# criteo/tf-yarn

Measured on AMD Instinct MI355X. Metric: examples/sec (whole node), Criteo wide-and-deep, higher is better.
Workload: dtype bf16; 1 GPU; model=wide_and_deep_criteo, global_batch=65536, per_gpu_batch=65536, dense_features=13, sparse_features=26, embedding_dim=16, table_rows_per_feature=1000000, parallelism=dp1, alltoall_mode=unprobed

## Files before the change

setup.py:

```python

import os

os.environ.setdefault("PYTORCH_ROCM_ARCH", "gfx950")

from pybind11.setup_helpers import Pybind11Extension
from setuptools import find_packages, setup
from torch.utils.cpp_extension import (BuildExtension,
                                       CUDAExtension)

CSRC = os.path.join("tf_yarn_amd", "ops", "csrc")

kv_ext = Pybind11Extension(
    "tf_yarn_amd._kv_native",
    sources=[os.path.join("tf_yarn_amd", "csrc_kv", "kv_server.cpp")],
    cxx_std=17,
    extra_compile_args=["-O2", "-pthread"],
)

ext = CUDAExtension(
    name="tf_yarn_amd.ops._C",
    sources=[
        os.path.join(CSRC, "bindings.cpp"),
        os.path.join(CSRC, "fused_optimizers.hip"),
        os.path.join(CSRC, "embedding.hip"),
        os.path.join(CSRC, "binned_scatter.hip"),
        os.path.join(CSRC, "sparse_adagrad.hip"),
        os.path.join(CSRC, "elementwise.hip"),
        os.path.join(CSRC, "wgrad.hip"),
        os.path.join(CSRC, "gemm_bt.hip"),
        os.path.join(CSRC, "lt_linear.hip"),
        os.path.join(CSRC, "eval_metrics.hip"),
    ],
    extra_compile_args={
        "cxx": ["-O3"],
        "nvcc": ["-O3", "--offload-arch=gfx950"],
    },
    libraries=["hipblaslt"],
)

setup(
    name="tf_yarn_amd",
    version="0.1.0",
    description=("MI355X-native distributed-training launcher with "
                 "criteo/tf-yarn's capabilities"),
    packages=find_packages(include=["tf_yarn_amd", "tf_yarn_amd.*"]),
    package_data={"tf_yarn_amd": ["default.log.conf"]},
    python_requires=">=3.9",
    ext_modules=[ext, kv_ext],
    cmdclass={"build_ext": BuildExtension},
)
```

tf_yarn_amd/models/wide_deep.py:

```python

from __future__ import annotations

import logging
import math
from typing import List, NamedTuple, Optional, Tuple

import torch
import torch.distributed as dist
from torch import nn

from tf_yarn_amd import ops

logger = logging.getLogger(__name__)

CRITEO_DENSE = 13
CRITEO_SPARSE = 26
DEFAULT_TABLE_SIZES = [1_000_000] * CRITEO_SPARSE


SPARSE_OPTIMIZERS = ("sgd", "adagrad", "ftrl")
DEEP_SPARSE_OPTIMIZERS = SPARSE_OPTIMIZERS + ("rowwise_adagrad",)


def _check_sparse_rule(name: str, value: str, dim: int = 1) -> str:
# ... 343 lines not shown
                                all_ids.reshape(all_grads.numel(), -1),
                                all_grads, alpha=-lr / world)
        self._gathered = []

    @torch.no_grad()
    def apply_sparse_updates(self, lr: float, process_group=None) -> None:
        if not self._sink:
            return
        self.start_sparse_sync(process_group)
        self.finish_sparse_sync(lr)

    def clear_pending(self) -> None:
        self._sink.clear()
        self._gathered = []


class _DeepInput(torch.autograd.Function):

    DENSE_PAD = 16

    @staticmethod
    def forward(ctx, dense, table, flat_ids, dim, out_bf16, sink):
        b = dense.shape[0]
        f = flat_ids.numel() // b
        dtype = torch.bfloat16 if out_bf16 else torch.float32
        out = torch.empty(b, _DeepInput.DENSE_PAD + f * dim,
                          dtype=dtype, device=dense.device)
        out[:, :dense.shape[1]] = dense.to(dtype)
        out[:, dense.shape[1]:_DeepInput.DENSE_PAD] = 0
        ops.emb_fwd_into(table, flat_ids, out, _DeepInput.DENSE_PAD)
        ctx.sink = sink
        ctx.save_for_backward(flat_ids)
        return out

    @staticmethod
    def backward(ctx, grad_out):
        (flat_ids,) = ctx.saved_tensors
        emb_grad = grad_out[:, _DeepInput.DENSE_PAD:].contiguous()
        ctx.sink.append((flat_ids, emb_grad))
        return None, None, None, None, None, None


class ScalarHead(nn.Module):

    def __init__(self, in_features: int, dtype=torch.float32):
        super().__init__()
        bound = 1.0 / math.sqrt(in_features)
        self.weight = nn.Parameter(
            (torch.rand(in_features, dtype=torch.float32) * 2 - 1) * bound)
        self.bias = nn.Parameter(torch.zeros(1, dtype=torch.float32))
        if dtype != torch.float32:
            self.weight.data = self.weight.data.to(dtype)
            self.bias.data = self.bias.data.to(dtype)

    def forward(self, x):
        if x.size(-1) % 4 == 0:
            return ops.ScalarHeadFn.apply(x, self.weight, self.bias)
        if x.is_cuda:
            pad = (-x.size(-1)) % 4
            xp = nn.functional.pad(x, (0, pad))
            wp = nn.functional.pad(self.weight, (0, pad))
            return ops.ScalarHeadFn.apply(xp, wp, self.bias)
        return x @ self.weight + self.bias


class FusedLinearReLU(nn.Module):

    def __init__(self, in_features: int, out_features: int,
                 dtype=torch.float32):
        super().__init__()
        self.weight = nn.Parameter(
            torch.empty(out_features, in_features, dtype=dtype))
        self.bias = nn.Parameter(torch.zeros(out_features, dtype=dtype))
        nn.init.kaiming_uniform_(self.weight, a=math.sqrt(5))

    def forward(self, x):
        return ops.linear_bias_relu(x, self.weight, self.bias)


class WideAndDeep(nn.Module):

    def __init__(self,
                 dense_dim: int = CRITEO_DENSE,
                 table_sizes: Optional[List[int]] = None,
                 embedding_dim: int = 16,
                 hidden: Tuple[int, ...] = (1024, 512, 256),
                 compute_dtype: torch.dtype = torch.float32,
                 sharded: bool = False,
                 process_group=None,
                 sparse_optimizer: str = "sgd",
                 sparse_eps: float = 1e-10,
                 sparse_initial_accumulator: float = 0.0,
                 wide_sparse_optimizer: Optional[str] = None,
                 sparse_l1: float = 0.0, sparse_l2: float = 0.0,
                 wide_sparse_lr: Optional[float] = None):
        super().__init__()
        table_sizes = table_sizes or DEFAULT_TABLE_SIZES
        if wide_sparse_optimizer is None:
            wide_sparse_optimizer = _default_wide_rule(sparse_optimizer)
        sparse_kw = dict(
            sparse_optimizer=sparse_optimizer, sparse_eps=sparse_eps,
            sparse_initial_accumulator=sparse_initial_accumulator,
            sparse_l1=sparse_l1, sparse_l2=sparse_l2)
        self.sparse_optimizer = sparse_optimizer
        self.wide_sparse_optimizer = wide_sparse_optimizer
        self.compute_dtype = compute_dtype
        self.dense_dim = dense_dim
        bf16 = compute_dtype == torch.bfloat16
        self.sharded = sharded
        if sharded:
            from tf_yarn_amd.models.sharded_embedding import \
                ShardedCriteoEmbeddings
            self.embeddings = ShardedCriteoEmbeddings(
                table_sizes, embedding_dim, out_bf16=bf16,
                process_group=process_group,
                wide_sparse_optimizer=wide_sparse_optimizer,
                wide_sparse_lr=wide_sparse_lr, **sparse_kw)
            self.deep_embedding = None
            self.wide_embedding = None
        else:
            self.embeddings = None
            self.deep_embedding = SparseEmbedding(
                table_sizes, embedding_dim, out_bf16=bf16, **sparse_kw)
            wide_kw = dict(sparse_kw, sparse_optimizer=wide_sparse_optimizer,
                           wide_sparse_lr=wide_sparse_lr)
            self.wide_embedding = WideScalarEmbedding(table_sizes,
                                                      out_bf16=bf16,
                                                      **wide_kw)
        self.wide_dense = ScalarHead(dense_dim, compute_dtype)
        layers: List[nn.Module] = []
        in_dim = _DeepInput.DENSE_PAD + len(table_sizes) * embedding_dim
        for h in hidden:
            layers.append(FusedLinearReLU(in_dim, h))
            in_dim = h
        self.mlp = nn.Sequential(*layers)
        self.head = ScalarHead(in_dim, compute_dtype)
        if bf16:
            self.mlp = self.mlp.to(torch.bfloat16)

    def _deep_tower(self, deep_in: torch.Tensor) -> torch.Tensor:
        n = len(self.mlp)
        last = self.mlp[n - 1] if n else None
        head = self.head
        if not (isinstance(last, FusedLinearReLU) and deep_in.is_cuda
                and ops.HAVE_EXT and deep_in.dim() == 2
                and deep_in.dtype == torch.bfloat16
                and last.weight.dtype == torch.bfloat16
                and last.bias.dtype == torch.bfloat16
                and head.weight.dtype == torch.bfloat16
                and head.bias.dtype == torch.bfloat16
                and last.weight.shape[0] % 4 == 0
                and ops.fused_head_bwd_enabled()):
            return head(self.mlp(deep_in))
        h = deep_in
        for i in range(n - 1):
            h = self.mlp[i](h)
        return ops.linear_bias_relu_head(h, last.weight, last.bias,
                                         head.weight, head.bias)

    def forward(self, dense: torch.Tensor, sparse_ids: torch.Tensor,
                labels: Optional[torch.Tensor] = None) -> torch.Tensor:
        dense = dense.to(self.compute_dtype)
        if self.sharded:
            b = dense.shape[0]
            emb = self.embeddings
            deep_in = torch.empty(
                b, _DeepInput.DENSE_PAD + emb.F * emb.dim,
                dtype=self.compute_dtype, device=dense.device)
            deep_in, wide_sum = emb(sparse_ids, deep_in,
                                    _DeepInput.DENSE_PAD, dense=dense)
            deep_out = self._deep_tower(deep_in)
            wide_sum = wide_sum.to(deep_out.dtype)
            wd = self.wide_dense(dense)
            if labels is not None:
                return ops.bce_head_loss(deep_out, wide_sum, wd, labels)
            return deep_out + wide_sum + wd
        emb = self.deep_embedding
        flat = (sparse_ids + emb.offsets.unsqueeze(0)).reshape(-1)
        deep_in = _DeepInput.apply(
            dense, emb.weight, flat, emb.dim,
            self.compute_dtype == torch.bfloat16, emb._sink)
        deep_out = self._deep_tower(deep_in)
        wide_emb = self.wide_embedding(sparse_ids).to(deep_out.dtype)
        wd = self.wide_dense(dense)
        if labels is not None:
            return ops.bce_head_loss(deep_out, wide_emb, wd, labels)
        return deep_out + wide_emb + wd

    def start_sparse_sync(self, process_group=None) -> None:
        if self.sharded:
            return
        self.deep_embedding.start_sparse_sync(process_group)
        self.wide_embedding.start_sparse_sync(process_group)

    def finish_sparse_sync(self, lr: float, stream=None) -> None:
        if self.sharded:
            self.embeddings.apply_sparse_updates(lr, stream=stream)
            return
        self.deep_embedding.finish_sparse_sync(lr)
        self.wide_embedding.finish_sparse_sync(lr)

    def apply_sparse_updates(self, lr: float, process_group=None) -> None:
        self.start_sparse_sync(process_group)
        self.finish_sparse_sync(lr)

    def clear_pending(self) -> None:
        if self.sharded:
            self.embeddings.clear_pending()
            return
        self.deep_embedding.clear_pending()
        self.wide_embedding.clear_pending()


class FlatInputWideAndDeep(nn.Module):

    def __init__(self, dense_dim: int = CRITEO_DENSE,
                 table_sizes: Optional[List[int]] = None,
                 embedding_dim: int = 16,
                 hidden: Tuple[int, ...] = (1024, 512, 256),
                 compute_dtype: torch.dtype = torch.float32,
                 sharded: bool = False, process_group=None,
                 sparse_optimizer: str = "sgd", sparse_eps: float = 1e-10,
                 sparse_initial_accumulator: float = 0.0,
                 wide_sparse_optimizer: Optional[str] = None,
                 sparse_l1: float = 0.0, sparse_l2: float = 0.0,
                 wide_sparse_lr: Optional[float] = None):
        super().__init__()
        self.dense_dim = dense_dim
        init_acc = sparse_initial_accumulator
        self.net = WideAndDeep(dense_dim=dense_dim,
                               sparse_optimizer=sparse_optimizer,
                               sparse_eps=sparse_eps,
                               sparse_initial_accumulator=init_acc,
                               wide_sparse_optimizer=wide_sparse_optimizer,
                               sparse_l1=sparse_l1, sparse_l2=sparse_l2,
                               wide_sparse_lr=wide_sparse_lr,
                               table_sizes=table_sizes,
                               embedding_dim=embedding_dim, hidden=hidden,
                               compute_dtype=compute_dtype,
                               sharded=sharded,
                               process_group=process_group)

    def forward(self, x: torch.Tensor,
                labels: Optional[torch.Tensor] = None) -> torch.Tensor:
        dense = x[:, :self.dense_dim]
        ids = x[:, self.dense_dim:].long()
        return self.net(dense, ids, labels=labels)

    def start_sparse_sync(self, process_group=None) -> None:
        self.net.start_sparse_sync(process_group)

    def finish_sparse_sync(self, lr: float, stream=None) -> None:
        self.net.finish_sparse_sync(lr, stream=stream)

    def apply_sparse_updates(self, lr: float, process_group=None) -> None:
        self.net.apply_sparse_updates(lr, process_group)

    def clear_pending(self) -> None:
        self.net.clear_pending()
```

tf_yarn_amd/ops/__init__.py:

```python

from __future__ import annotations

import functools
import logging
import os
from typing import NamedTuple, Optional, Tuple

import torch

logger = logging.getLogger(__name__)

try:
    from tf_yarn_amd.ops import _C
    HAVE_EXT = True
except ImportError as _e:
    _C = None
    HAVE_EXT = False
    _IMPORT_ERROR = _e


def _require_ext() -> None:
    if not HAVE_EXT:
        raise RuntimeError(
            "tf_yarn_amd.ops._C is not built but a GPU tensor was passed. "
# ... 696 lines not shown
    return _env_switch_on("MIYARN_FUSED_HEAD_GRADS")


def col_reduce_dot_sum(x: torch.Tensor, dy: torch.Tensor,
                       out_dtype: torch.dtype = torch.float32):
    if _on_gpu(x, dy):
        _require_ext()
        if out_dtype in (torch.float32, torch.bfloat16):
            dw, db = _C.col_reduce_dot_sum(x.contiguous(), dy.contiguous(),
                                           out_dtype == torch.bfloat16)
            return dw, db
        dw, db = _C.col_reduce_dot_sum(x.contiguous(), dy.contiguous(),
                                       False)
        return dw.to(out_dtype), db.to(out_dtype)
    dw = (x.float() * dy.float().unsqueeze(1)).sum(dim=0)
    db = dy.float().sum().reshape(1)
    return dw.to(out_dtype), db.to(out_dtype)


def row_dot(x: torch.Tensor, w: torch.Tensor,
            bias: "torch.Tensor | None" = None) -> torch.Tensor:
    if _on_gpu(x, w) and x.size(1) % 4 == 0 and x.size(1) <= 512:
        _require_ext()
        return _C.row_dot(x.contiguous(), w.contiguous(), bias)
    y = x @ w
    return y if bias is None else y + bias


def gemm_bt(a: torch.Tensor, b: torch.Tensor,
            bias: "torch.Tensor | None" = None,
            relu: bool = False) -> torch.Tensor:
    if _on_gpu(a, b):
        _require_ext()
        return _C.gemm_bt(a.contiguous(), b.contiguous(), bias, relu)
    out = a.float() @ b.float().t()
    if bias is not None:
        out = out + bias.float()
    if relu:
        out = torch.relu(out)
    return out.to(a.dtype)


class ScalarHeadFn(torch.autograd.Function):

    @staticmethod
    def forward(ctx, x, weight, bias):
        ctx.save_for_backward(x, weight)
        if _on_gpu(x, weight) and x.size(1) % 4 == 0 \
                and x.size(1) <= 512 and bias.numel() == 1:
            _require_ext()
            return _C.row_dot(x.contiguous(), weight.contiguous(),
                              bias.reshape(1))
        return x @ weight + bias

    @staticmethod
    def backward(ctx, dy):
        x, weight = ctx.saved_tensors
        dy = dy.contiguous()
        dx = dw = db = None
        if ctx.needs_input_grad[0]:
            dx = dy.unsqueeze(1) * weight.unsqueeze(0)
        if ctx.needs_input_grad[1] and ctx.needs_input_grad[2] \
                and _on_gpu(x, dy) and x.dtype == dy.dtype \
                and fused_head_grads_enabled():
            dw, db = col_reduce_dot_sum(x, dy, weight.dtype)
            return dx, dw, db
        if ctx.needs_input_grad[1]:
            dw = col_reduce_dot(x, dy).to(weight.dtype)
        if ctx.needs_input_grad[2]:
            db = dy.sum().reshape(1).to(weight.dtype)
        return dx, dw, db


class BCEHeadFn(torch.autograd.Function):

    @staticmethod
    def forward(ctx, deep, wide, dhead, labels):
        if deep.is_cuda and HAVE_EXT and deep.dtype == torch.bfloat16 \
                and wide.dtype == torch.bfloat16 \
                and dhead.dtype == torch.bfloat16:
            loss, sig = _C.bce_head_fwd(
                deep.contiguous(), wide.contiguous(), dhead.contiguous(),
                labels.contiguous().float())
        else:
            z = (deep.float() + wide.float() + dhead.float())
            labels = labels.float()
            loss = torch.nn.functional.binary_cross_entropy_with_logits(
                z, labels, reduction="none")
            sig = torch.sigmoid(z).to(deep.dtype)
        ctx.save_for_backward(sig, labels)
        ctx.dtype = deep.dtype
        return loss

    @staticmethod
    def backward(ctx, g):
        sig, labels = ctx.saved_tensors
        if sig.is_cuda and HAVE_EXT and sig.dtype == torch.bfloat16:
            dl = _C.bce_head_bwd(sig, labels.contiguous().float(),
                                 g.contiguous().float())
        else:
            dl = ((sig.float() - labels.float()) * g.float()).to(ctx.dtype)
        return dl, dl, dl, None


def bce_head_loss(deep: torch.Tensor, wide: torch.Tensor,
                  dhead: torch.Tensor, labels: torch.Tensor) -> torch.Tensor:
    return BCEHeadFn.apply(deep, wide, dhead, labels).mean()


class BiasReLU(torch.autograd.Function):

    @staticmethod
    def forward(ctx, x, bias):
        y = bias_relu_fwd(x, bias)
        ctx.save_for_backward(y)
        return y

    @staticmethod
    def backward(ctx, dy):
        (y,) = ctx.saved_tensors
        if dy.is_cuda and HAVE_EXT and y.size(-1) % 4 == 0 \
                and y.size(-1) <= 8192:
            dx, dbias = _C.bias_relu_bwd_db(
                dy.contiguous(), y.contiguous(),
                dy.dtype == torch.bfloat16)
            return dx, dbias.to(dy.dtype)
        dx = bias_relu_bwd(dy.contiguous(), y)
        dims = tuple(range(dx.dim() - 1))
        dbias = dx.sum(dim=dims)
        return dx, dbias


def bias_relu(x: torch.Tensor, bias: torch.Tensor) -> torch.Tensor:
    return BiasReLU.apply(x, bias)


def _custom_wgrad_kernel(dz: torch.Tensor, x: torch.Tensor):
    if os.environ.get("MIYARN_WGRAD") == "lib":
        return None
    if not (dz.is_cuda and HAVE_EXT):
        return None
    if dz.dtype != torch.bfloat16 or x.dtype != torch.bfloat16:
        return None
    n, m = dz.size(1), x.size(1)
    if m % 8 != 0 or dz.size(0) % 64 != 0:
        return None
    if n % 256 == 0 and n * m > 256 * 512:
        return _C.wgrad_nt256
    if n % 128 == 0 and n * m <= 256 * 512:
        return _C.wgrad_nt128
    return None


def _custom_fwd_ok(x: torch.Tensor, weight: torch.Tensor,
                   bias: torch.Tensor) -> bool:
    if os.environ.get("MIYARN_FWD") != "custom":
        return False
    if not (x.is_cuda and HAVE_EXT):
        return False
    if x.dtype != torch.bfloat16 or weight.dtype != torch.bfloat16 \
            or bias.dtype != torch.bfloat16:
        return False
    if x.dim() != 2 or not x.is_contiguous() or not weight.is_contiguous():
        return False
    m, k = x.shape
    return m % 256 == 0 and k % 16 == 0 and weight.size(0) % 16 == 0


def _lt_fwd_ok(x, weight, bias) -> bool:
    if os.environ.get("MIYARN_LT_FWD", "1") in ("", "0"):
        return False
    return (x.is_cuda and HAVE_EXT and x.dim() == 2
            and x.dtype == torch.bfloat16
            and weight.dtype == torch.bfloat16
            and bias.dtype == torch.bfloat16
            and x.is_contiguous() and weight.is_contiguous())


def _linear_bias_relu_fwd(x: torch.Tensor, weight: torch.Tensor,
                          bias: torch.Tensor) -> torch.Tensor:
    if _custom_fwd_ok(x, weight, bias):
        return _C.gemm_bt(x, weight, bias, True)
    if _lt_fwd_ok(x, weight, bias):
        return _C.lt_linear(x, weight, bias.contiguous(), True)
    return bias_relu_fwd(x.matmul(weight.t()), bias)


def _linear_wgrad(dz: torch.Tensor, x: torch.Tensor,
                  weight: torch.Tensor) -> torch.Tensor:
    kernel = _custom_wgrad_kernel(dz, x)
    if kernel is None:
        return dz.t().matmul(x)
    dw = kernel(dz, x, 0, weight.dtype == torch.bfloat16)
    return dw if dw.dtype == weight.dtype else dw.to(weight.dtype)


class LinearBiasReLU(torch.autograd.Function):

    @staticmethod
    def forward(ctx, x, weight, bias):
        y = _linear_bias_relu_fwd(x, weight, bias)
        ctx.save_for_backward(x, weight, y)
        return y

    @staticmethod
    def backward(ctx, dy):
        x, weight, y = ctx.saved_tensors
        dy = dy.contiguous()
        if dy.is_cuda and HAVE_EXT and y.size(-1) % 4 == 0 \
                and y.size(-1) <= 8192:
            dz, dbias = _C.bias_relu_bwd_db(
                dy, y.contiguous(), dy.dtype == torch.bfloat16)
            if dbias.dtype != dy.dtype:
                dbias = dbias.to(dy.dtype)
        else:
            dz = bias_relu_bwd(dy, y)
            dbias = dz.sum(dim=tuple(range(dz.dim() - 1)))
        dx = dz.matmul(weight)
        return dx, _linear_wgrad(dz, x, weight), dbias


def linear_bias_relu(x: torch.Tensor, weight: torch.Tensor,
                     bias: torch.Tensor) -> torch.Tensor:
    return LinearBiasReLU.apply(x, weight, bias)



def fused_head_bwd_enabled() -> bool:
    return _env_switch_on("MIYARN_FUSED_HEAD_BWD")


def head_relu_bwd_db(dl: torch.Tensor, w_head: torch.Tensor,
                     y: torch.Tensor):
    if _on_gpu(dl, w_head, y) and HAVE_EXT and dl.dtype == y.dtype \
            and w_head.dtype == y.dtype and y.dim() == 2 \
            and y.size(1) % 4 == 0 and y.size(1) <= 8192:
        dz, dbias = _C.head_relu_bwd_db(
            dl.contiguous(), w_head.contiguous(), y.contiguous(),
            y.dtype == torch.bfloat16)
        return dz, dbias.to(y.dtype)
    if _on_gpu(dl, w_head, y):
        _require_ext()
    dz = bias_relu_bwd(dl.unsqueeze(1) * w_head.unsqueeze(0), y)
    return dz, dz.sum(dim=0)


def head_relu_bwd_grads(dl: torch.Tensor, w_head: torch.Tensor,
                        y: torch.Tensor):
    if _on_gpu(dl, w_head, y) and HAVE_EXT and dl.dtype == y.dtype \
            and w_head.dtype == y.dtype and y.dim() == 2 \
            and y.size(1) % 4 == 0 and y.size(1) <= 8192 \
            and y.dtype in (torch.float32, torch.bfloat16):
        dz, dbias, dw_head, db_head = _C.head_relu_bwd_grads(
            dl.contiguous(), w_head.contiguous(), y.contiguous(),
            y.dtype == torch.bfloat16)
        return dz, dbias, dw_head, db_head
    dw_head = col_reduce_dot(y, dl).to(w_head.dtype)
    db_head = dl.sum().reshape(1).to(w_head.dtype)
    dz, dbias = head_relu_bwd_db(dl, w_head, y)
    return dz, dbias, dw_head, db_head


class LinearBiasReLUHeadFn(torch.autograd.Function):

    @staticmethod
    def forward(ctx, x, weight, bias, w_head, b_head):
        y = _linear_bias_relu_fwd(x, weight, bias)
        ctx.save_for_backward(x, weight, y, w_head)
        if _on_gpu(y, w_head) and y.size(1) % 4 == 0 \
                and y.size(1) <= 512 and b_head.numel() == 1:
            _require_ext()
            return _C.row_dot(y.contiguous(), w_head.contiguous(),
                              b_head.reshape(1))
        return y @ w_head + b_head

    @staticmethod
    def backward(ctx, dl):
        x, weight, y, w_head = ctx.saved_tensors
        dl = dl.contiguous()
        dw_head = db_head = None
        if ctx.needs_input_grad[3] and ctx.needs_input_grad[4] \
                and _on_gpu(dl, y) and fused_head_grads_enabled():
            dz, dbias, dw_head, db_head = head_relu_bwd_grads(dl, w_head, y)
        else:
            if ctx.needs_input_grad[3]:
                dw_head = col_reduce_dot(y, dl).to(w_head.dtype)
            if ctx.needs_input_grad[4]:
                db_head = dl.sum().reshape(1).to(w_head.dtype)
            dz, dbias = head_relu_bwd_db(dl, w_head, y)
        dx = dz.matmul(weight)
        dw = _linear_wgrad(dz, x, weight)
        return dx, dw, dbias, dw_head, db_head


def linear_bias_relu_head(x: torch.Tensor, weight: torch.Tensor,
                          bias: torch.Tensor, w_head: torch.Tensor,
                          b_head: torch.Tensor) -> torch.Tensor:
    return LinearBiasReLUHeadFn.apply(x, weight, bias, w_head, b_head)



EVAL_BUCKETS = 4096
EVAL_SLOTS = 256


class BinaryEvalState:

    def __init__(self, device=None):
        self.hist = torch.zeros(2, EVAL_BUCKETS, dtype=torch.int64,
                                device=device)
        self.counts = torch.zeros(4, dtype=torch.int64, device=device)
        self.sums = torch.zeros(EVAL_SLOTS, 2, dtype=torch.float64,
                                device=device)

    def tensors(self) -> Tuple[torch.Tensor, torch.Tensor, torch.Tensor]:
        return self.hist, self.counts, self.sums

    def zero_(self) -> "BinaryEvalState":
        for t in self.tensors():
            t.zero_()
        return self


def _binary_eval_update_ref(z: torch.Tensor, y: torch.Tensor,
                            state: BinaryEvalState) -> None:
    nan = torch.isnan(z) | torch.isnan(y)
    n_nan = int(nan.sum())
    z, y = z[~nan], y[~nan]
    pos = y >= 0.5
    hot = z > 0
    t = (z + 16.0) * 128.0
    k = torch.floor(t).clamp_(0.0, EVAL_BUCKETS - 1.0).to(torch.int64)
    state.hist[0] += torch.bincount(k[~pos], minlength=EVAL_BUCKETS)
    state.hist[1] += torch.bincount(k[pos], minlength=EVAL_BUCKETS)
    state.counts += torch.tensor(
        [z.numel(), n_nan, int((pos & hot).sum()), int((~pos & hot).sum())],
        dtype=torch.int64)
    loss = z.clamp_min(0.0) - z * y + torch.log1p(torch.exp(-z.abs()))
    sig = 1.0 / (1.0 + torch.exp(-z))
    state.sums[0, 0] += loss.double().sum()
    state.sums[0, 1] += sig.double().sum()


def binary_eval_update(logits: torch.Tensor, labels: torch.Tensor,
                       state: BinaryEvalState) -> None:
    z = logits.reshape(-1)
    y = labels.reshape(-1)
    if z.numel() != y.numel():
        raise ValueError(f"{z.numel()} logits but {y.numel()} labels")
    if y.dtype != torch.float32:
        y = y.float()
    if z.numel() == 0:
        return
    if _on_gpu(z, y, *state.tensors()):
        _require_ext()
        if z.dtype not in (torch.float32, torch.bfloat16):
            z = z.float()
        _C.binary_eval_update(z.contiguous(), y.contiguous(),
                              *state.tensors())
        return
    _binary_eval_update_ref(z.float(), y, state)
```

tf_yarn_amd/ops/csrc/bindings.cpp:

```cpp
#include <torch/extension.h>
#include <string>
#include <tuple>
#include <vector>

void fused_sgd(torch::Tensor param, torch::Tensor grad,
               c10::optional<torch::Tensor> momentum_buf,
               c10::optional<torch::Tensor> param_bf16,
               double lr, double momentum, double dampening,
               double weight_decay, bool nesterov, bool first_step,
               double grad_scale);
void fused_sgd_mt(std::vector<torch::Tensor> params,
                  std::vector<torch::Tensor> grads,
                  std::vector<torch::Tensor> momentum_bufs,
                  std::vector<torch::Tensor> params_bf16,
                  double lr, double momentum, double dampening,
                  double weight_decay, bool nesterov, bool first_step,
                  double grad_scale);
void fused_adam(torch::Tensor param, torch::Tensor grad,
                torch::Tensor exp_avg, torch::Tensor exp_avg_sq,
                c10::optional<torch::Tensor> param_bf16,
                double lr, double beta1, double beta2, double eps,
                double weight_decay, bool adamw, int64_t step,
                double grad_scale);
void fused_adagrad(torch::Tensor param, torch::Tensor grad,
                   torch::Tensor state_sum, double lr, double eps,
                   double weight_decay, double grad_scale);
void fused_ftrl(torch::Tensor param, torch::Tensor grad,
                torch::Tensor accum, torch::Tensor linear, double lr,
                double l1, double l2, double grad_scale);
void fused_adadelta(torch::Tensor param, torch::Tensor grad,
                    torch::Tensor square_avg, torch::Tensor acc_delta,
                    double lr, double rho, double eps, double weight_decay,
                    double grad_scale);

torch::Tensor emb_fwd(torch::Tensor table, torch::Tensor ids, bool out_bf16);
void emb_bwd_sgd(torch::Tensor table, torch::Tensor ids, torch::Tensor grad,
                 double lr, double scale);
void emb_bwd_sgd_sorted(torch::Tensor table, torch::Tensor sorted_ids,
                        torch::Tensor grad, double lr, double scale);
void emb_bwd_dense(torch::Tensor grad_table, torch::Tensor ids,
                   torch::Tensor grad, double scale);
void emb_bwd_sgd_fused_wide_offs(torch::Tensor table,
                                 torch::Tensor wide_table, torch::Tensor ids,
                                 torch::Tensor grad, torch::Tensor gw,
                                 double lr, double scale,
                                 c10::optional<torch::Tensor> offsets);
bool emb_lookup_fused_ok(int64_t dim, int64_t n_features, int64_t n_dense,
                         int64_t col_offset, int64_t out_cols);
torch::Tensor emb_lookup_fused(torch::Tensor table, torch::Tensor wide_table,
                               torch::Tensor ids, torch::Tensor offsets,
                               c10::optional<torch::Tensor> dense,
                               torch::Tensor out, int64_t col_offset);

torch::Tensor emb_gather_sum(torch::Tensor table, torch::Tensor ids,
                             int64_t batch, bool out_bf16);
void emb_fwd_into(torch::Tensor table, torch::Tensor ids,
                  torch::Tensor out, int64_t col_offset);
void emb_scatter_sum(torch::Tensor table, torch::Tensor ids,
                     torch::Tensor grad, double alpha);

using SparseSide = std::tuple<std::string, torch::Tensor,
                              std::vector<torch::Tensor>, torch::Tensor,
                              c10::optional<torch::Tensor>, double, double,
                              double, double>;
void emb_bwd_sparse(c10::optional<SparseSide> deep,
                    c10::optional<SparseSide> wide, torch::Tensor stamp,
                    torch::Tensor ids, int64_t epoch, double scale);
bool sparse_pair_fused_ok(const std::string& deep_rule,
                          const std::string& wide_rule, int64_t dim);
py::dict binned_layout();
std::vector<torch::Tensor> binned_permutation(torch::Tensor ids,
                                              int64_t n_rows,
                                              int64_t region_bits);
void emb_bwd_sgd_binned(torch::Tensor table, torch::Tensor ids,
                        torch::Tensor grad, double lr, double scale,
                        torch::Tensor order, torch::Tensor starts);
void emb_scatter_sum_binned(torch::Tensor table, torch::Tensor ids,
                            torch::Tensor grad, int64_t g_div,
                            double alpha, torch::Tensor order,
                            torch::Tensor starts);

torch::Tensor bias_relu_fwd(torch::Tensor x, torch::Tensor bias);
torch::Tensor bias_relu_bwd(torch::Tensor dy, torch::Tensor y);
std::vector<torch::Tensor> bias_relu_bwd_db(torch::Tensor dy,
                                            torch::Tensor y,
                                            bool dbias_bf16);
std::vector<torch::Tensor> head_relu_bwd_db(torch::Tensor dl,
                                            torch::Tensor w_head,
                                            torch::Tensor y,
                                            bool dbias_bf16);
std::vector<torch::Tensor> head_relu_bwd_grads(torch::Tensor dl,
                                               torch::Tensor w_head,
                                               torch::Tensor y,
                                               bool out_bf16);
torch::Tensor reduce_splitk(torch::Tensor part, bool out_bf16);
torch::Tensor reduce_tall(torch::Tensor part, bool out_bf16,
                          int64_t quad_lanes);

torch::Tensor lt_linear(torch::Tensor x, torch::Tensor w,
                        c10::optional<torch::Tensor> bias, bool relu);
torch::Tensor col_reduce_dot(torch::Tensor x, torch::Tensor dy);
std::vector<torch::Tensor> col_reduce_dot_sum(torch::Tensor x,
                                              torch::Tensor dy,
                                              bool out_bf16);
torch::Tensor row_dot(torch::Tensor x, torch::Tensor w,
                      c10::optional<torch::Tensor> bias);
std::vector<torch::Tensor> bce_head_fwd(torch::Tensor deep,
                                        torch::Tensor wide,
                                        torch::Tensor dhead,
                                        torch::Tensor labels);
torch::Tensor bce_head_bwd(torch::Tensor sig, torch::Tensor labels,
                           torch::Tensor g);

torch::Tensor wgrad_nt128(torch::Tensor dy, torch::Tensor x,
                          int64_t splitk, bool out_bf16);
torch::Tensor wgrad_nt256(torch::Tensor dy, torch::Tensor x,
                          int64_t splitk, bool out_bf16);
void convert_scaled(torch::Tensor src, torch::Tensor dst, double scale);

torch::Tensor gemm_bt(torch::Tensor a, torch::Tensor b,
                      c10::optional<torch::Tensor> bias, bool relu);

void binary_eval_update(torch::Tensor logits, torch::Tensor labels,
                        torch::Tensor hist, torch::Tensor counts,
                        torch::Tensor sums);

PYBIND11_MODULE(TORCH_EXTENSION_NAME, m) {
  m.doc() = "tf_yarn_amd MI355X (gfx950) HIP kernels";
  m.def("fused_sgd", &fused_sgd, "Fused SGD(+momentum) step");
  m.def("fused_sgd_mt", &fused_sgd_mt,
        "Multi-tensor fused SGD (one launch per <=24 tensors)");
  m.def("fused_adam", &fused_adam, "Fused Adam/AdamW step");
  m.def("fused_adagrad", &fused_adagrad, "Fused Adagrad step");
  m.def("fused_adadelta", &fused_adadelta, "Fused Adadelta step");
  m.def("emb_fwd", &emb_fwd, "Fused multi-table embedding gather");
  m.def("emb_bwd_sgd", &emb_bwd_sgd,
        "Fused sparse embedding grad scatter + SGD update");
  m.def("emb_bwd_sgd_sorted", &emb_bwd_sgd_sorted,
        "Atomic-free segmented scatter+SGD over SORTED ids");
  m.def("emb_bwd_sgd_fused_wide", &emb_bwd_sgd_fused_wide_offs,
        "Fused deep scatter+SGD + wide scalar scatter (shared ids; with "
        "offsets, raw [batch, features] ids)",
        py::arg("table"), py::arg("wide_table"), py::arg("ids"),
        py::arg("grad"), py::arg("gw"), py::arg("lr"), py::arg("scale"),
        py::arg("offsets") = py::none());
  m.def("emb_lookup_fused_ok", &emb_lookup_fused_ok,
        "Whether emb_lookup_fused covers (dim, features, n_dense, "
        "col_offset, out_cols)");
  m.def("emb_lookup_fused", &emb_lookup_fused,
        "Offset add + deep gather into a slice + wide gather-sum + dense/"
        "pad columns in one kernel (returns the wide sums)",
        py::arg("table"), py::arg("wide_table"), py::arg("ids"),
        py::arg("offsets"), py::arg("dense"), py::arg("out"),
        py::arg("col_offset"));
  m.def("emb_bwd_dense", &emb_bwd_dense,
        "Sparse embedding grad scatter into dense grad table");
  m.def("emb_bwd_sparse", &emb_bwd_sparse,
        "Stateful sparse update (adagrad, ftrl, rowwise_adagrad) of a deep "
        "side, a wide side or both from shared ids: atomic accumulate + "
        "once-per-row claim/apply; sides without gradients run the apply "
        "alone on their accumulators",
        py::arg("deep"), py::arg("wide"), py::arg("stamp"), py::arg("ids"),
        py::arg("epoch"), py::arg("scale"));
  m.def("sparse_pair_fused_ok", &sparse_pair_fused_ok,
        "Whether emb_bwd_sparse has a fused deep+wide kernel for (deep rule, "
        "wide rule, deep dim)");
  m.def("fused_ftrl", &fused_ftrl, "Fused dense FTRL-proximal step");
  m.def("bias_relu_fwd", &bias_relu_fwd, "Fused bias+ReLU forward");
  m.def("bias_relu_bwd", &bias_relu_bwd, "Fused ReLU backward");
  m.def("lt_linear", &lt_linear,
        "hipBLASLt linear with fused bias(+ReLU) epilogue",
        py::arg("x"), py::arg("w"), py::arg("bias") = py::none(),
        py::arg("relu") = false);
  m.def("reduce_splitk", &reduce_splitk,
        "Split-K partial reduction with fused output cast",
        py::arg("part"), py::arg("out_bf16") = false);
  m.def("reduce_tall", &reduce_tall,
        "reduce_splitk's tall-slab kernel with 1 or 4 quad lanes per block",
        py::arg("part"), py::arg("out_bf16") = false,
        py::arg("quad_lanes") = 1);
  m.def("wgrad_nt128", &wgrad_nt128,
        "Split-K MFMA weight gradient dW = dy^T @ x (bf16 in), 128x128 tiles",
        py::arg("dy"), py::arg("x"), py::arg("splitk"),
        py::arg("out_bf16") = false);
  m.def("wgrad_nt256", &wgrad_nt256,
        "Split-K MFMA weight gradient dW = dy^T @ x (bf16 in), 256x256 tiles",
        py::arg("dy"), py::arg("x"), py::arg("splitk"),
        py::arg("out_bf16") = false);
  m.def("col_reduce_dot", &col_reduce_dot,
        "dw[m] = sum_b dy[b] * x[b,m] (single-logit head wgrad)");
  m.def("col_reduce_dot_sum", &col_reduce_dot_sum,
        "col_reduce_dot plus db = sum_b dy[b] from the same pass "
        "(returns [dw, db])",
        py::arg("x"), py::arg("dy"), py::arg("out_bf16") = false);
  m.def("row_dot", &row_dot,
        "y[b] = x[b].w + bias (single-logit head forward GEMV)");
  m.def("bce_head_fwd", &bce_head_fwd,
        "Fused 3-part logit sum + stable BCEWithLogits (loss, sigmoid)");
  m.def("bce_head_bwd", &bce_head_bwd,
        "dlogit = (sigmoid - label) * upstream grad");
  m.def("bias_relu_bwd_db", &bias_relu_bwd_db,
        "Fused ReLU backward + dbias reduction (returns [dx, dbias])",
        py::arg("dy"), py::arg("y"), py::arg("dbias_bf16") = false);
  m.def("head_relu_bwd_db", &head_relu_bwd_db,
        "ReLU backward + dbias of the layer under a single-logit head, from "
        "dl and w_head (no outer product; returns [dz, dbias])",
        py::arg("dl"), py::arg("w_head"), py::arg("y"),
        py::arg("dbias_bf16") = false);
  m.def("head_relu_bwd_grads", &head_relu_bwd_grads,
        "head_relu_bwd_db plus the head's own dw and db from the same pass "
        "(returns [dz, dbias, dw_head, db_head])",
        py::arg("dl"), py::arg("w_head"), py::arg("y"),
        py::arg("out_bf16") = false);
  m.def("emb_fwd_into", &emb_fwd_into,
        "Embedding gather into a slice of a larger 2D buffer");
  m.def("emb_gather_sum", &emb_gather_sum,
        "Wide-part gather-sum: out[b] = sum_f table[ids[b,f]]");
  m.def("binned_layout", &binned_layout,
        "Layout constants of the binned scatter (hash capacities, probe "
        "limit, hash threshold, launch shapes)");
  m.def("binned_permutation", &binned_permutation,
        "Region-binned permutation of sparse update indices");
  m.def("emb_bwd_sgd_binned", &emb_bwd_sgd_binned,
        "Binned LDS-dedup scatter+SGD (deep tables, dim=16)");
  m.def("emb_scatter_sum_binned", &emb_scatter_sum_binned,
        "Binned LDS-dedup scatter-add (scalar wide tables)");
  m.def("emb_scatter_sum", &emb_scatter_sum,
        "Wide-part scatter: table[ids[b,f]] += alpha * g[b]");
  m.def("convert_scaled", &convert_scaled, "Scaled bf16<->fp32 convert");
  m.def("gemm_bt", &gemm_bt,
        "C = A @ B^T (both K-major bf16) with fused bias+ReLU epilogue");
  m.def("binary_eval_update", &binary_eval_update,
        "Fold a batch of (logit, label) into the streaming binary eval "
        "state: score histogram [2, 4096], counts (n_valid, n_nan, tp, fp), "
        "per-slot fp64 (loss, sigmoid) sums [256, 2]",
        py::arg("logits"), py::arg("labels"), py::arg("hist"),
        py::arg("counts"), py::arg("sums"));
}
```

Baseline: 59.08 million examples/s.

## Fuse hidden-layer dgrad GEMM with ReLU backward and dbias reduction

Adds a HIP MFMA kernel that computes dz_next @ W and applies the ReLU mask of the layer below in the epilogue. It also accumulates per-tile column sums for dbias. A new whole-MLP autograd function routes selected layer shapes through this kernel during backward. The goal is to avoid materialising and re-reading the unmasked dgrad output and to cut kernel launches. The cost is a hand-written GEMM that may be less efficient than the library GEMM, plus a split-k reduction for dbias.

```diff
diff --git a/setup.py b/setup.py
--- a/setup.py
+++ b/setup.py
@@ -28,6 +28,7 @@
         os.path.join(CSRC, "elementwise.hip"),
         os.path.join(CSRC, "wgrad.hip"),
         os.path.join(CSRC, "gemm_bt.hip"),
+        os.path.join(CSRC, "dgrad_drelu.hip"),
         os.path.join(CSRC, "lt_linear.hip"),
         os.path.join(CSRC, "eval_metrics.hip"),
     ],
diff --git a/tf_yarn_amd/models/wide_deep.py b/tf_yarn_amd/models/wide_deep.py
--- a/tf_yarn_amd/models/wide_deep.py
+++ b/tf_yarn_amd/models/wide_deep.py
@@ -519,6 +519,14 @@
                 and last.weight.shape[0] % 4 == 0
                 and ops.fused_head_bwd_enabled()):
             return head(self.mlp(deep_in))
+        if all(isinstance(m, FusedLinearReLU)
+               and m.weight.dtype == torch.bfloat16
+               and m.bias.dtype == torch.bfloat16 for m in self.mlp):
+            weights = [m.weight for m in self.mlp]
+            if ops.mlp_head_routed(deep_in, weights):
+                return ops.mlp_bias_relu_head(
+                    deep_in, weights, [m.bias for m in self.mlp],
+                    head.weight, head.bias)
         h = deep_in
         for i in range(n - 1):
             h = self.mlp[i](h)
diff --git a/tf_yarn_amd/ops/__init__.py b/tf_yarn_amd/ops/__init__.py
--- a/tf_yarn_amd/ops/__init__.py
+++ b/tf_yarn_amd/ops/__init__.py
@@ -872,6 +872,13 @@
     return None
 
 
+def _fused_dgrad_shape_routed(k: int, n: int) -> bool:
+    return (k, n) in _FUSED_DGRAD_SHAPES
+
+
+_FUSED_DGRAD_SHAPES = frozenset({(256, 512), (512, 1024)})
+
+
 def _custom_fwd_ok(x: torch.Tensor, weight: torch.Tensor,
                    bias: torch.Tensor) -> bool:
     if os.environ.get("MIYARN_FWD") != "custom":
@@ -1017,6 +1024,118 @@
                           bias: torch.Tensor, w_head: torch.Tensor,
                           b_head: torch.Tensor) -> torch.Tensor:
     return LinearBiasReLUHeadFn.apply(x, weight, bias, w_head, b_head)
+
+
+
+def fused_dgrad_enabled() -> bool:
+    return _env_switch_on("MIYARN_FUSED_DGRAD")
+
+
+def _dgrad_drelu_kernel_ok(dz_next: torch.Tensor, weight: torch.Tensor,
+                           y: torch.Tensor) -> bool:
+    if not (HAVE_EXT and dz_next.is_cuda and weight.is_cuda and y.is_cuda):
+        return False
+    if not (dz_next.dtype == weight.dtype == y.dtype == torch.bfloat16):
+        return False
+    if not (dz_next.dim() == 2 and weight.dim() == 2 and y.dim() == 2):
+        return False
+    m, k = dz_next.shape
+    n = weight.shape[1]
+    return (weight.shape[0] == k and tuple(y.shape) == (m, n) and m > 0
+            and m % 256 == 0 and k % 16 == 0 and n % 16 == 0)
+
+
+def dgrad_drelu(dz_next: torch.Tensor, weight: torch.Tensor,
+                y: torch.Tensor):
+    if _dgrad_drelu_kernel_ok(dz_next, weight, y):
+        dz, dbias = _C.dgrad_drelu(dz_next.contiguous(),
+                                   weight.contiguous(), y.contiguous(),
+                                   True)
+        return dz, dbias
+    return _relu_bwd_db(dz_next.matmul(weight), y)
+
+
+def _relu_bwd_db(dy: torch.Tensor, y: torch.Tensor):
+    dy = dy.contiguous()
+    if dy.is_cuda and HAVE_EXT and y.size(-1) % 4 == 0 \
+            and y.size(-1) <= 8192:
+        dz, dbias = _C.bias_relu_bwd_db(
+            dy, y.contiguous(), dy.dtype == torch.bfloat16)
+        if dbias.dtype != dy.dtype:
+            dbias = dbias.to(dy.dtype)
+        return dz, dbias
+    dz = bias_relu_bwd(dy, y)
+    return dz, dz.sum(dim=tuple(range(dz.dim() - 1)))
+
+
+class MLPHeadFn(torch.autograd.Function):
+
+    @staticmethod
+    def forward(ctx, x, w_head, b_head, *wb):
+        n = len(wb) // 2
+        weights, biases = wb[:n], wb[n:]
+        ys = []
+        h = x
+        for w, b in zip(weights, biases):
+            h = _linear_bias_relu_fwd(h, w, b)
+            ys.append(h)
+        ctx.n_layers = n
+        ctx.save_for_backward(x, w_head, *weights, *ys)
+        if _on_gpu(h, w_head) and h.size(1) % 4 == 0 \
+                and h.size(1) <= 512 and b_head.numel() == 1:
+            _require_ext()
+            return _C.row_dot(h.contiguous(), w_head.contiguous(),
+                              b_head.reshape(1))
+        return h @ w_head + b_head
+
+    @staticmethod
+    def backward(ctx, dl):
+        n = ctx.n_layers
+        saved = ctx.saved_tensors
+        x, w_head = saved[0], saved[1]
+        weights, ys = saved[2:2 + n], saved[2 + n:]
+        dl = dl.contiguous()
+        dw_head = db_head = None
+        if ctx.needs_input_grad[1] and ctx.needs_input_grad[2] \
+                and _on_gpu(dl, ys[-1]) and fused_head_grads_enabled():
+            dz, dbias, dw_head, db_head = head_relu_bwd_grads(
+                dl, w_head, ys[-1])
+        else:
+            if ctx.needs_input_grad[1]:
+                dw_head = col_reduce_dot(ys[-1], dl).to(w_head.dtype)
+            if ctx.needs_input_grad[2]:
+                db_head = dl.sum().reshape(1).to(w_head.dtype)
+            dz, dbias = head_relu_bwd_db(dl, w_head, ys[-1])
+        dws = [None] * n
+        dbs = [None] * n
+        fused = fused_dgrad_enabled()
+        for l in range(n - 1, 0, -1):
+            w, y_below = weights[l], ys[l - 1]
+            dws[l] = _linear_wgrad(dz, y_below, w)
+            dbs[l] = dbias
+            if fused and _fused_dgrad_shape_routed(*w.shape) \
+                    and _dgrad_drelu_kernel_ok(dz, w, y_below):
+                dz, dbias = dgrad_drelu(dz, w, y_below)
+            else:
+                dz, dbias = _relu_bwd_db(dz.matmul(w), y_below)
+        dx = dz.matmul(weights[0]) if ctx.needs_input_grad[0] else None
+        dws[0] = _linear_wgrad(dz, x, weights[0])
+        dbs[0] = dbias
+        return (dx, dw_head, db_head, *dws, *dbs)
+
+
+def mlp_bias_relu_head(x: torch.Tensor, weights, biases,
+                       w_head: torch.Tensor,
+                       b_head: torch.Tensor) -> torch.Tensor:
+    return MLPHeadFn.apply(x, w_head, b_head, *weights, *biases)
+
+
+def mlp_head_routed(x: torch.Tensor, weights) -> bool:
+    if not (fused_dgrad_enabled() and x.dim() == 2 and x.size(0) > 0
+            and x.size(0) % 256 == 0):
+        return False
+    return any(_fused_dgrad_shape_routed(*w.shape) and w.shape[0] % 16 == 0
+               and w.shape[1] % 16 == 0 for w in weights[1:])
 
 
 
diff --git a/tf_yarn_amd/ops/csrc/bindings.cpp b/tf_yarn_amd/ops/csrc/bindings.cpp
--- a/tf_yarn_amd/ops/csrc/bindings.cpp
+++ b/tf_yarn_amd/ops/csrc/bindings.cpp
@@ -120,6 +120,9 @@
 
 torch::Tensor gemm_bt(torch::Tensor a, torch::Tensor b,
                       c10::optional<torch::Tensor> bias, bool relu);
+
+std::vector<torch::Tensor> dgrad_drelu(torch::Tensor dz_next, torch::Tensor w,
+                                       torch::Tensor y, bool dbias_bf16);
 
 void binary_eval_update(torch::Tensor logits, torch::Tensor labels,
                         torch::Tensor hist, torch::Tensor counts,
@@ -230,6 +233,11 @@
   m.def("convert_scaled", &convert_scaled, "Scaled bf16<->fp32 convert");
   m.def("gemm_bt", &gemm_bt,
         "C = A @ B^T (both K-major bf16) with fused bias+ReLU epilogue");
+  m.def("dgrad_drelu", &dgrad_drelu,
+        "Hidden-layer dgrad dz_next @ w with the ReLU backward of the layer "
+        "below and its dbias in the epilogue (returns [dz, dbias])",
+        py::arg("dz_next"), py::arg("w"), py::arg("y"),
+        py::arg("dbias_bf16") = false);
   m.def("binary_eval_update", &binary_eval_update,
         "Fold a batch of (logit, label) into the streaming binary eval "
         "state: score histogram [2, 4096], counts (n_valid, n_nan, tp, fp), "
diff --git a/tf_yarn_amd/ops/csrc/dgrad_drelu.hip b/tf_yarn_amd/ops/csrc/dgrad_drelu.hip
--- /dev/null
+++ b/tf_yarn_amd/ops/csrc/dgrad_drelu.hip
@@ -0,0 +1,283 @@
+
+#include <torch/extension.h>
+#include <c10/hip/HIPStream.h>
+#include "mfma_tile.h"
+
+torch::Tensor reduce_splitk(torch::Tensor part, bool out_bf16);
+
+namespace {
+
+#define DD_BK 64
+#define DD_TILE 128
+
+union DdU16x4 {
+  unsigned short u[4];
+  unsigned long long ll;
+};
+
+template <int PW>
+__device__ __forceinline__ int park_off(int row, int col) {
+  constexpr int CPR = PW / 8;
+  constexpr int RP = 256 / (PW * 2);
+  const int chunk = (col >> 3) ^ ((row / RP) & (CPR - 1));
+  return row * (PW * 2) + (chunk << 4) + (col & 7) * 2;
+}
+
+template <int TILE>
+__global__ __launch_bounds__(2 * TILE, 2)
+void dgrad_drelu_kernel(const unsigned short* __restrict__ A,
+                        const unsigned short* __restrict__ W,
+                        const unsigned short* __restrict__ Y,
+                        unsigned short* __restrict__ DZ,
+                        float* __restrict__ part,
+                        int64_t M, int N, int K) {
+  constexpr int FI = 4;
+  constexpr int FJ = TILE / 32;
+  constexpr int SC = TILE / 8;
+  constexpr int NW = TILE / 32;
+  constexpr int PW = TILE / 2;
+  constexpr int OPR = PW / 8;
+  constexpr int RPS = 2 * TILE / OPR;
+  constexpr int SW = TILE / RPS;
+
+  const int tiles_n = (N + TILE - 1) / TILE;
+  const int tiles_m = static_cast<int>(M / TILE);
+  int tile_m, tile_n;
+  if ((tiles_m & 7) == 0) {
+    const int c = blockIdx.x & 7;
+    const int q = blockIdx.x >> 3;
+    tile_n = q % tiles_n;
+    tile_m = c + 8 * (q / tiles_n);
+  } else {
+    tile_m = blockIdx.x / tiles_n;
+    tile_n = blockIdx.x - tile_m * tiles_n;
+  }
+  const int64_t m0 = (int64_t)tile_m * TILE;
+  const int n0 = tile_n * TILE;
+
+  __shared__ __attribute__((aligned(16))) unsigned char
+      lds_raw[2 * TILE * 128];
+  unsigned char* aT = lds_raw;
+  unsigned char* wT = lds_raw + TILE * 128;
+
+  const int tid = threadIdx.x;
+  const int lane = tid & 63;
+  const int wave = tid >> 6;
+  const int wm = (wave >> 1) * 64;
+  const int wn = (wave & 1) * (TILE / 2);
+
+  const int st_r = tid >> 1;
+  const int st_k = (tid & 1) * 32;
+  const int st_kg = (tid / SC) * 4;
+  const int st_c = (tid % SC) * 8;
+  const bool w_col_ok = (n0 + st_c) < N;
+
+  mfma_f32x4 acc[FI][FJ];
+#pragma unroll
+  for (int i = 0; i < FI; ++i)
+#pragma unroll
+    for (int j = 0; j < FJ; ++j) acc[i][j] = {0.f, 0.f, 0.f, 0.f};
+
+  const int a_row = lane & 15;
+  const int a_k = (lane >> 4) * 8;
+
+  bf16x8 ra[4], rw[4];
+
+  auto load_step = [&](int k0) {
+    const unsigned short* pa = A + (m0 + st_r) * (int64_t)K + k0 + st_k;
+#pragma unroll
+    for (int c = 0; c < 4; ++c) {
+      ra[c] = bf16x8{0, 0, 0, 0, 0, 0, 0, 0};
+      if (k0 + st_k + c * 8 + 8 <= K)
+        ra[c] = *reinterpret_cast<const bf16x8*>(pa + c * 8);
+    }
+    const bool w_ok = w_col_ok && (k0 + st_kg) < K;
+#pragma unroll
+    for (int rr = 0; rr < 4; ++rr) {
+      rw[rr] = bf16x8{0, 0, 0, 0, 0, 0, 0, 0};
+      if (w_ok)
+        rw[rr] = *reinterpret_cast<const bf16x8*>(
+            W + (int64_t)(k0 + st_kg + rr) * N + n0 + st_c);
+    }
+  };
+
+  auto write_step = [&] {
+#pragma unroll
+    for (int c = 0; c < 4; ++c)
+      *reinterpret_cast<bf16x8*>(aT + lds_off_linear(st_r, st_k + c * 8)) =
+          ra[c];
+#pragma unroll
+    for (int j = 0; j < 8; ++j) {
+      DdU16x4 p{{rw[0][j], rw[1][j], rw[2][j], rw[3][j]}};
+      *reinterpret_cast<unsigned long long*>(
+          wT + lds_off(st_c + j, st_kg)) = p.ll;
+    }
+  };
+
+  const int e_m = lane & 15;
+  const int e_n = (lane >> 4) * 4;
+  const int w_row = tid / OPR;
+  const int w_oct = tid - w_row * OPR;
+
+  bf16x8 yv[2][SW];
+  auto load_y = [&] {
+#pragma unroll
+    for (int p = 0; p < 2; ++p) {
+      const int col = n0 + p * PW + w_oct * 8;
+#pragma unroll
+      for (int s = 0; s < SW; ++s) {
+        yv[p][s] = bf16x8{0, 0, 0, 0, 0, 0, 0, 0};
+        if (col < N)
+          yv[p][s] = *reinterpret_cast<const bf16x8*>(
+              Y + (m0 + s * RPS + w_row) * (int64_t)N + col);
+      }
+    }
+  };
+
+  load_step(0);
+  for (int k0 = 0; k0 < K; k0 += DD_BK) {
+    write_step();
+    __syncthreads();
+    if (k0 + DD_BK < K) load_step(k0 + DD_BK);
+#pragma unroll
+    for (int kh = 0; kh < 2; ++kh) {
+      mfma_bf16x8 a[FI], b[FJ];
+#pragma unroll
+      for (int i = 0; i < FI; ++i)
+        a[i] = *reinterpret_cast<const mfma_bf16x8*>(
+            aT + lds_off_linear(wm + i * 16 + a_row, kh * 32 + a_k));
+#pragma unroll
+      for (int j = 0; j < FJ; ++j)
+        b[j] = *reinterpret_cast<const mfma_bf16x8*>(
+            wT + lds_off(wn + j * 16 + a_row, kh * 32 + a_k));
+#pragma unroll
+      for (int i = 0; i < FI; ++i)
+#pragma unroll
+        for (int j = 0; j < FJ; ++j)
+          acc[i][j] = __builtin_amdgcn_mfma_f32_16x16x32_bf16(
+              b[j], a[i], acc[i][j], 0, 0, 0);
+    }
+    __syncthreads();
+  }
+
+  load_y();
+
+  float cs[2][8];
+#pragma unroll
+  for (int p = 0; p < 2; ++p)
+#pragma unroll
+    for (int j = 0; j < 8; ++j) cs[p][j] = 0.f;
+
+#pragma unroll
+  for (int p = 0; p < 2; ++p) {
+    if ((wave & 1) == p) {
+#pragma unroll
+      for (int i = 0; i < FI; ++i)
+#pragma unroll
+        for (int j = 0; j < FJ; ++j) {
+          DdU16x4 v{{f32_to_bf16(acc[i][j][0]), f32_to_bf16(acc[i][j][1]),
+                     f32_to_bf16(acc[i][j][2]), f32_to_bf16(acc[i][j][3])}};
+          *reinterpret_cast<unsigned long long*>(
+              lds_raw + park_off<PW>(wm + i * 16 + e_m, j * 16 + e_n)) =
+              v.ll;
+        }
+    }
+    __syncthreads();
+    const int col = n0 + p * PW + w_oct * 8;
+#pragma unroll
+    for (int s = 0; s < SW; ++s) {
+      const int row = s * RPS + w_row;
+      const bf16x8 cv = *reinterpret_cast<const bf16x8*>(
+          lds_raw + park_off<PW>(row, w_oct * 8));
+      bf16x8 out;
+#pragma unroll
+      for (int j = 0; j < 8; ++j) {
+        const bool keep = bf16_to_f32(yv[p][s][j]) > 0.f;
+        out[j] = keep ? cv[j] : (unsigned short)0;
+        if (keep) cs[p][j] += bf16_to_f32(cv[j]);
+      }
+      if (col < N)
+        *reinterpret_cast<bf16x8*>(DZ + (m0 + row) * (int64_t)N + col) = out;
+    }
+    __syncthreads();
+  }
+
+  float* fsum = reinterpret_cast<float*>(lds_raw);
+#pragma unroll
+  for (int p = 0; p < 2; ++p) {
+#pragma unroll
+    for (int j = 0; j < 8; ++j) {
+      float v = cs[p][j];
+#pragma unroll
+      for (int off = OPR; off < 64; off <<= 1) v += __shfl_xor(v, off);
+      cs[p][j] = v;
+    }
+    if (lane < OPR) {
+      float* dst = fsum + wave * TILE + p * PW + lane * 8;
+      reinterpret_cast<f32x4*>(dst)[0] =
+          f32x4{cs[p][0], cs[p][1], cs[p][2], cs[p][3]};
+      reinterpret_cast<f32x4*>(dst)[1] =
+          f32x4{cs[p][4], cs[p][5], cs[p][6], cs[p][7]};
+    }
+  }
+  __syncthreads();
+  if (tid < TILE && n0 + tid < N) {
+    float s = 0.f;
+#pragma unroll
+    for (int w = 0; w < NW; ++w) s += fsum[w * TILE + tid];
+    part[(int64_t)tile_m * N + n0 + tid] = s;
+  }
+}
+
+template <int TILE>
+std::vector<torch::Tensor> dgrad_drelu_launch(const torch::Tensor& dz_next,
+                                              const torch::Tensor& w,
+                                              const torch::Tensor& y,
+                                              bool dbias_bf16) {
+  const int64_t M = dz_next.size(0);
+  const int K = static_cast<int>(dz_next.size(1));
+  const int N = static_cast<int>(w.size(1));
+  auto dz = torch::empty({M, (int64_t)N}, y.options());
+  auto part = torch::empty({M / TILE, (int64_t)N},
+                           y.options().dtype(torch::kFloat32));
+  auto stream = c10::hip::getCurrentHIPStream().stream();
+  dim3 grid((M / TILE) * ((N + TILE - 1) / TILE));
+  hipLaunchKernelGGL(
+      dgrad_drelu_kernel<TILE>, grid, dim3(2 * TILE), 0, stream,
+      reinterpret_cast<const unsigned short*>(dz_next.data_ptr()),
+      reinterpret_cast<const unsigned short*>(w.data_ptr()),
+      reinterpret_cast<const unsigned short*>(y.data_ptr()),
+      reinterpret_cast<unsigned short*>(dz.data_ptr()),
+      part.data_ptr<float>(), M, N, K);
+  return {dz, reduce_splitk(part, dbias_bf16)};
+}
+
+}
+
+std::vector<torch::Tensor> dgrad_drelu(torch::Tensor dz_next, torch::Tensor w,
+                                       torch::Tensor y, bool dbias_bf16) {
+  TORCH_CHECK(dz_next.is_cuda() && dz_next.is_contiguous() &&
+              dz_next.dim() == 2 &&
+              dz_next.scalar_type() == torch::kBFloat16,
+              "dz_next must be [M, K] bf16 contiguous");
+  TORCH_CHECK(w.is_cuda() && w.is_contiguous() && w.dim() == 2 &&
+              w.scalar_type() == torch::kBFloat16,
+              "w must be [K, N] bf16 contiguous");
+  TORCH_CHECK(y.is_cuda() && y.is_contiguous() && y.dim() == 2 &&
+              y.scalar_type() == torch::kBFloat16,
+              "y must be [M, N] bf16 contiguous");
+  const int64_t M = dz_next.size(0);
+  const int64_t K = dz_next.size(1);
+  const int64_t N = w.size(1);
+  TORCH_CHECK(w.size(0) == K, "K mismatch");
+  TORCH_CHECK(y.size(0) == M && y.size(1) == N, "y must be [M, N]");
+  TORCH_CHECK(dz_next.device() == w.device() && w.device() == y.device(),
+              "operands on different devices");
+  TORCH_CHECK(M > 0 && M % 256 == 0 && N > 0 && N % 16 == 0 && K > 0 &&
+              K % 16 == 0,
+              "dgrad_drelu needs M % 256 == 0, N % 16 == 0, K % 16 == 0");
+  TORCH_CHECK(N < (1 << 30) && K < (1 << 30) &&
+              (M / 128) * ((N + 127) / 128) < (1LL << 31),
+              "dgrad_drelu: shape too large");
+  return dgrad_drelu_launch<DD_TILE>(dz_next, w, y, dbias_bf16);
+}
```

Measured after the change: 62.36 million examples/s, median of 6. 5.6% higher.
